# alibaba/nann

Measured on AMD Instinct MI355X. Metric: retrieval QPS @ recall@200 parity, 1M items/128-d, higher is better.
Workload: dtype f16 rows / f32 L2

## Files before the change

### nann_amd/csrc/nann_device.h

```cpp
#pragma once
#include <type_traits>
#include <hip/hip_runtime.h>
#include <hip/hip_fp16.h>
#include <stdint.h>

namespace nann {

constexpr int kNT = 1024;
constexpr int kNW = kNT / 64;
constexpr int kTopkEPT = 16;
constexpr int kMaxK = 1024;
constexpr int kPhaseScratch = 27648;
constexpr int kMaxD = 512;
constexpr int kLdsScoresOff = 10752;
constexpr int kLdsScores = 4096;

enum : int { DT_F16 = 0, DT_BF16 = 1, DT_F32 = 2 };

__device__ __forceinline__ int local_tid() {
  int t = threadIdx.x;
  asm volatile("" : "+v"(t));
  __builtin_assume(t >= 0 && t < 1024);
  return t;
}
// ... 775 lines not shown

template <int DT>
struct RowChunk {
  uint4 a;
  uint4 b;
};

template <int DT>
__device__ __forceinline__ RowChunk<DT> load_chunk(const void* table, size_t row, int d, int sub) {
  RowChunk<DT> r;
  if constexpr (DT == DT_F32) {
    const uint4* p = reinterpret_cast<const uint4*>(static_cast<const float*>(table) + row * d + sub * 8);
    r.a = p[0];
    r.b = p[1];
  } else {
    const uint4* p = reinterpret_cast<const uint4*>(static_cast<const uint16_t*>(table) + row * d + sub * 8);
    r.a = p[0];
    r.b = make_uint4(0, 0, 0, 0);
  }
  return r;
}

template <int DT>
__device__ __forceinline__ void chunk_to_float(const RowChunk<DT>& r, float x[8]) {
  if constexpr (DT == DT_F32) {
    x[0] = __uint_as_float(r.a.x); x[1] = __uint_as_float(r.a.y);
    x[2] = __uint_as_float(r.a.z); x[3] = __uint_as_float(r.a.w);
    x[4] = __uint_as_float(r.b.x); x[5] = __uint_as_float(r.b.y);
    x[6] = __uint_as_float(r.b.z); x[7] = __uint_as_float(r.b.w);
  } else {
    const uint32_t w[4] = {r.a.x, r.a.y, r.a.z, r.a.w};
#pragma unroll
    for (int i = 0; i < 4; ++i) {
      if constexpr (DT == DT_F16) {
        x[2 * i] = half_bits_to_float(w[i] & 0xffffu);
        x[2 * i + 1] = half_bits_to_float(w[i] >> 16);
      } else {
        x[2 * i] = bf16_bits_to_float(w[i] & 0xffffu);
        x[2 * i + 1] = bf16_bits_to_float(w[i] >> 16);
      }
    }
  }
}

template <int LPR>
__device__ __forceinline__ float l2_finish(const float q[8], const float x[8]) {
  float acc = 0.0f;
#pragma unroll
  for (int k = 0; k < 8; ++k) {
    const float t = q[k] - x[k];
    acc = __fmaf_rn(t, t, acc);
  }
  acc = acc + dpp_f32<0xB1>(acc);
  acc = acc + dpp_f32<0x4E>(acc);
  if constexpr (LPR >= 8) acc = acc + dpp_f32<0x141>(acc);
  if constexpr (LPR >= 16) acc = acc + dpp_f32<0x140>(acc);
  if constexpr (LPR >= 32) acc = acc + __shfl_xor(acc, 16);
  if constexpr (LPR >= 64) acc = acc + __shfl_xor(acc, 32);
  return 0.0f - acc;
}

__device__ __forceinline__ float l2_lane_f16(const float q[8], const uint4& a) {
  const uint32_t w[4] = {a.x, a.y, a.z, a.w};
  float acc = 0.0f;
#pragma unroll
  for (int i = 0; i < 4; ++i) {
    float t0, t1;
    asm("v_fma_mix_f32 %0, %1, -1.0, %2 op_sel_hi:[1,0,0]" : "=v"(t0) : "v"(w[i]), "v"(q[2 * i]));
    asm("v_fma_mix_f32 %0, %1, -1.0, %2 op_sel:[1,0,0] op_sel_hi:[1,0,0]" : "=v"(t1) : "v"(w[i]), "v"(q[2 * i + 1]));
    acc = __fmaf_rn(t0, t0, acc);
    acc = __fmaf_rn(t1, t1, acc);
  }
  return acc;
}
__device__ __forceinline__ float l2_lane_bf16(const float q[8], const uint4& a) {
  const uint32_t w[4] = {a.x, a.y, a.z, a.w};
  float acc = 0.0f;
#pragma unroll
  for (int i = 0; i < 4; ++i) {
    const float t0 = q[2 * i] - __uint_as_float(w[i] << 16);
    const float t1 = q[2 * i + 1] - __uint_as_float(w[i] & 0xffff0000u);
    acc = __fmaf_rn(t0, t0, acc);
    acc = __fmaf_rn(t1, t1, acc);
  }
  return acc;
}
__device__ __forceinline__ float l2_rows8_reduce_scatter(float (&a)[8]) {
  float t0, t1, t2, t3;
  asm("s_mov_b32 vcc_lo, 0x5a5a5a5a\n\ts_mov_b32 vcc_hi, 0x5a5a5a5a\n\t"
      "v_cndmask_b32_e32 %8, %0, %1, vcc\n\tv_cndmask_b32_e32 %0, %1, %0, vcc\n\t"
      "v_cndmask_b32_e32 %9, %2, %3, vcc\n\tv_cndmask_b32_e32 %2, %3, %2, vcc\n\t"
      "v_cndmask_b32_e32 %10, %4, %5, vcc\n\tv_cndmask_b32_e32 %4, %5, %4, vcc\n\t"
      "v_cndmask_b32_e32 %11, %6, %7, vcc\n\tv_cndmask_b32_e32 %6, %7, %6, vcc\n\t"
      "v_add_f32_dpp %8, %0, %8 quad_perm:[1,0,3,2] row_mask:0xf bank_mask:0xf\n\t"
      "v_add_f32_dpp %9, %2, %9 quad_perm:[1,0,3,2] row_mask:0xf bank_mask:0xf\n\t"
      "v_add_f32_dpp %10, %4, %10 quad_perm:[1,0,3,2] row_mask:0xf bank_mask:0xf\n\t"
      "v_add_f32_dpp %11, %6, %11 quad_perm:[1,0,3,2] row_mask:0xf bank_mask:0xf\n\t"
      "s_mov_b32 vcc_lo, 0x3c3c3c3c\n\ts_mov_b32 vcc_hi, 0x3c3c3c3c\n\t"
      "v_cndmask_b32_e32 %1, %9, %8, vcc\n\tv_cndmask_b32_e32 %3, %11, %10, vcc\n\t"
      "v_cndmask_b32_e32 %0, %8, %9, vcc\n\tv_cndmask_b32_e32 %2, %10, %11, vcc\n\t"
      "v_add_f32_dpp %0, %1, %0 quad_perm:[2,3,0,1] row_mask:0xf bank_mask:0xf\n\t"
      "v_add_f32_dpp %2, %3, %2 quad_perm:[2,3,0,1] row_mask:0xf bank_mask:0xf\n\t"
      "s_mov_b32 vcc_lo, 0x0ff00ff0\n\ts_mov_b32 vcc_hi, 0x0ff00ff0\n\t"
      "v_cndmask_b32_e32 %8, %2, %0, vcc\n\tv_cndmask_b32_e32 %9, %0, %2, vcc\n\t"
      "s_nop 0\n\t"
      "v_add_f32_dpp %9, %8, %9 row_half_mirror row_mask:0xf bank_mask:0xf\n\t"
      "s_nop 1\n\t"
      "v_add_f32_dpp %9, %9, %9 row_mirror row_mask:0xf bank_mask:0xf"
      : "+v"(a[0]), "+v"(a[1]), "+v"(a[2]), "+v"(a[3]), "+v"(a[4]), "+v"(a[5]), "+v"(a[6]), "+v"(a[7]),
        "=&v"(t0), "=&v"(t1), "=&v"(t2), "=&v"(t3)
      :
      : "vcc");
  return t1;
}

#ifndef NANN_SCORE_U
#define NANN_SCORE_U 8
#endif
#ifndef NANN_SCORE_NT
#define NANN_SCORE_NT 0
#endif
template <int LPR, int DT, int NWAVES>
__device__ __forceinline__ void wg_score_l2_part(const void* __restrict__ table, int d, const int32_t* ids,
                                                 int begin, int end, const float* qv, float* scores,
                                                 int wave_rel, bool near = false) {
  constexpr int U = (DT == DT_F32) ? NANN_SCORE_U / 2 : NANN_SCORE_U;
  constexpr int GPW = 64 / LPR;
  constexpr int RPI = NWAVES * GPW;
  if (end <= begin) return;
  const int lane = local_tid() & 63;
  const int sub = lane % LPR, grp = lane / LPR;
  const int slot = wave_rel * GPW + grp;
  float q[8];
#pragma unroll
  for (int k = 0; k < 8; ++k) q[k] = qv[sub * 8 + k];
  if constexpr (LPR >= 16 && DT != DT_F32) {
    static_assert(U == 8, "eight broadcasts below");
    constexpr uint32_t kRowBytes = LPR * 16;
    const int mine_at = (sub & (U - 1)) * RPI + slot;
    const int out_at = ((sub & 7) ^ ((sub & 4) ? 3 : 0)) * RPI + slot;
    auto run = [&](auto near_c) {
      constexpr bool NEAR = decltype(near_c)::value;
      auto row = [&](int32_t v) -> uint4 {
        if constexpr (NEAR) {
#if NANN_SCORE_NT
          typedef uint32_t u32x4_t __attribute__((ext_vector_type(4)));
          const u32x4_t r = __builtin_nontemporal_load(reinterpret_cast<const u32x4_t*>(static_cast<const unsigned char*>(table) + ((uint32_t)v | ((uint32_t)sub * 16u))));
          return uint4{r.x, r.y, r.z, r.w};
#else
          return *reinterpret_cast<const uint4*>(static_cast<const unsigned char*>(table) + ((uint32_t)v | ((uint32_t)sub * 16u)));
#endif
        } else {
          return load_chunk<DT>(table, (size_t)v, d, sub).a;
        }
      };
      auto widen = [&](int32_t id) -> int32_t { return NEAR ? (int32_t)__umul24((uint32_t)id, kRowBytes) : id; };
      auto ids_of = [&](int at) -> int32_t { return widen(ids[min(at + mine_at, end - 1)]); };
      int32_t idv = ids_of(begin);
      uint4 ch[U];
      ch[0] = row(dpp_i32<0x150>(idv));
      ch[1] = row(dpp_i32<0x151>(idv));
      ch[2] = row(dpp_i32<0x152>(idv));
      ch[3] = row(dpp_i32<0x153>(idv));
      ch[4] = row(dpp_i32<0x154>(idv));
      ch[5] = row(dpp_i32<0x155>(idv));
      ch[6] = row(dpp_i32<0x156>(idv));
      ch[7] = row(dpp_i32<0x157>(idv));
      idv = ids_of(begin + RPI * U);
      auto lane_sum = [&](const uint4& c) -> float { return DT == DT_F16 ? l2_lane_f16(q, c) : l2_lane_bf16(q, c); };
      auto finish = [&](float (&s)[U], int i0) {
        float mine = l2_rows8_reduce_scatter(s);
        if constexpr (LPR >= 32) mine = mine + __shfl_xor(mine, 16);
        if constexpr (LPR >= 64) mine = mine + __shfl_xor(mine, 32);
        const int i = i0 + out_at;
        if (sub < U && i < end) scores[i] = 0.0f - mine;
      };
      int i0 = begin;
      for (; i0 + RPI * U < end; i0 += RPI * U) {
        const int32_t idn = ids_of(i0 + 2 * RPI * U);
        float s[U];
#define NANN_ROLL_SLOT(u, ctrl)                 \
        s[u] = lane_sum(ch[u]);                     \
        ch[u] = row(dpp_i32<ctrl>(idv));            \
        __builtin_amdgcn_sched_barrier(0);
        NANN_ROLL_SLOT(0, 0x150) NANN_ROLL_SLOT(1, 0x151) NANN_ROLL_SLOT(2, 0x152) NANN_ROLL_SLOT(3, 0x153)
        NANN_ROLL_SLOT(4, 0x154) NANN_ROLL_SLOT(5, 0x155) NANN_ROLL_SLOT(6, 0x156) NANN_ROLL_SLOT(7, 0x157)
#undef NANN_ROLL_SLOT
        finish(s, i0);
        idv = idn;
      }
      {
        float s[U];
#pragma unroll
        for (int u = 0; u < U; ++u) s[u] = lane_sum(ch[u]);
        finish(s, i0);
      }
    };
    if (near) run(std::true_type{}); else run(std::false_type{});
    return;
  }
  int32_t nxt[U];
#pragma unroll
  for (int u = 0; u < U; ++u) nxt[u] = ids[min(begin + u * RPI + slot, end - 1)];
  for (int i0 = begin; i0 < end; i0 += RPI * U) {
    RowChunk<DT> ch[U];
#pragma unroll
    for (int u = 0; u < U; ++u) ch[u] = load_chunk<DT>(table, (size_t)nxt[u], d, sub);
#pragma unroll
    for (int u = 0; u < U; ++u)
      nxt[u] = ids[min(i0 + RPI * U + u * RPI + slot, end - 1)];
#pragma unroll
    for (int u = 0; u < U; ++u) {
      const int i = i0 + u * RPI + slot;
      float x[8];
      chunk_to_float<DT>(ch[u], x);
      const float s = l2_finish<LPR>(q, x);
      if (sub == 0 && i < end) scores[i] = s;
    }
  }
}

template <int LPR, int DT, int NTHREADS>
__device__ __forceinline__ void wg_score_l2(const void* __restrict__ table, int d, const int32_t* ids,
                                            int n, const float* qv, float* scores) {
  wg_score_l2_part<LPR, DT, NTHREADS / 64>(table, d, ids, 0, n, qv, scores, local_tid() >> 6);
}

template <int KCAP>
struct TopkScratchT {
  unsigned long long sel[KCAP < 512 ? 512 : KCAP];
  union {
    unsigned short prank[kNT];
    struct { uint32_t above[256]; uint32_t cursor[256]; } bins;
  };
  uint32_t misc[4];
  uint32_t wlo[kNW], whi[kNW];
  uint32_t wcnt[kNW];
};
static_assert(kNT * sizeof(unsigned short) == 512 * sizeof(uint32_t), "the bin tables overlay the partial ranks");
typedef TopkScratchT<kMaxK> TopkScratch;
static_assert(sizeof(TopkScratch) <= kLdsScoresOff, "top-k scratch overlaps the LDS scores");
static_assert(kLdsScoresOff + kLdsScores * 4 <= kPhaseScratch, "phase scratch too small");
static_assert(sizeof(ExpandWalkScratch) <= kPhaseScratch, "phase scratch too small");

template <int NS, bool SCL, int NT, int KCAP = kMaxK, bool BIN = false>
__device__ __forceinline__ int wg_topk_impl(const int32_t* ids, const float* scores,
                                            const float* lds_scores, int n, int k, int32_t* out_pos,
                                            int32_t* out_ids, float* out_scores, const int64_t* id_map,
                                            int64_t* out_mapped, unsigned char* scratch, SubTimer pt,
                                            int n_all = 0x7fffffff, uint32_t floor_key = 0u) {
  TopkScratchT<KCAP>* S = reinterpret_cast<TopkScratchT<KCAP>*>(scratch);
  long long tsub = pt.now();
  const int tid = local_tid(), lane = tid & 63, wave = tid >> 6;
  const uint64_t lt = lanemask_lt(lane);
  constexpr bool REG = NS > 0;
  uint32_t key[REG ? NS : 1];
  if constexpr (REG) {
    float raw[NS];
#pragma unroll
    for (int j = 0; j < NS; ++j) {
      const int i = min(j * NT + tid, n - 1);
      raw[j] = SCL ? lds_scores[i] : scores[i];
    }
#pragma unroll
    for (int j = 0; j < NS; ++j) key[j] = (j * NT + tid < n) ? score_key(raw[j]) : 0u;
  }
#define NANN_FOR_KEYS(...)                                                    \
  if constexpr (REG) {                                                        \
    _Pragma("unroll") for (int j = 0; j < NS; ++j) {                          \
      const int i = j * NT + tid;                                             \
      const uint32_t kj = key[j];                                             \
      const bool valid = i < n && (!BIN || i < n_all || kj > floor_key);      \
      __VA_ARGS__                                                             \
    }                                                                         \
  } else {                                                                    \
    for (int i0 = 0; i0 < n; i0 += NT) {                                      \
      const int i = i0 + tid;                                                 \
// ... 279 lines not shown
```

### nann_amd/csrc/nann_hip.hip

```cpp
#include "nann_eval.h"
#include "nann_attn.h"
#include "nann_order_kernels.h"
#include "host/nann_graphdef_text.h"
#include "host/nann_blaze_options.h"
#include "host/nann_npy.h"
#include "host/nann_projcache.h"

#include <algorithm>
#include <atomic>
#include <cmath>
#include <cstdio>
#include <cstdlib>
#include <cstring>
#include <fstream>
#include <memory>
#include <mutex>
#include <string>
#include <vector>

#include <sys/stat.h>

using namespace nann;

namespace nann {
// ... 2089 lines not shown
    if (cache) projection_used(*cache, tab, st);
    return r2;
  };
  if (attn) {
    a.attn = attn->P;
    if (tab) {
      auto launch = attn->precision == NANN_MLP_SPLIT_F16 ? launch_search_attn_proj : launch_search_attn_xproj;
      const bool resident = attn->precision == NANN_MLP_SPLIT_F16;
      return both([&](int vis, int, int slots, size_t lds) {
        if (resident && vis == VIS_LDS_HASH && !a.redo) return launch_search_attn_res(slots, lds, a, st);
        return launch(vis, slots, lds, a, st);
      });
    }
    auto launch = attn->precision == NANN_MLP_SPLIT_F16 ? launch_search_attn_split : launch_search_attn;
    return both([&](int vis, int, int slots, size_t lds) { return launch(ix->desc.d, dt, vis, slots, lds, a, st); });
  }
  a.mlp = scorer->mlp;
  a.phase = 0;
  const int exact = scorer->desc.kind == NANN_SCORER_MLP && scorer->desc.precision == NANN_MLP_EXACT_F32;
  if (mlp_res && p.phased) {
    DeviceInfo di;
    rc = device_info(&di);
    if (rc) return rc;
    const int k5 = level_topn[5];
    for (int64_t c0 = 0; c0 < n_queries && !rc; c0 += kPhaseChunk) {
      SearchArgs c = a;
      c.n_queries = (int)std::min<int64_t>(kPhaseChunk, n_queries - c0);
      c.q = q + (size_t)c0 * a.d;
      if (tq) c.tq = tq + (size_t)c0 * 6;
      c.out_ids = out_item_ids + (size_t)c0 * k5;
      if (out_scores) c.out_scores = out_scores + (size_t)c0 * k5;
      if (out_index) c.out_index = out_index + (size_t)c0 * k5;
      c.status = status + c0;
      if (counters) c.counters = counters + (size_t)c0 * 3 * NANN_NUM_ROUNDS;
      if (phase_ticks) c.phase_ticks = reinterpret_cast<long long*>(phase_ticks) + (size_t)c0 * NANN_NUM_PHASES;
      if (c0) HIP_TRY(hipMemsetAsync(workspace, 0, 256, st));
      const int slots = (int)std::min<int64_t>(c.n_queries, (int64_t)p.phase_slots);
      for (int ph = 0; ph <= NANN_NUM_ROUNDS && !rc; ++ph) {
        c.phase = ph;
        rc = launch_search_mlp_phase(p.phase_vis, slots, p.phase_lds_bytes, c, st);
        if (!rc && ph < NANN_NUM_ROUNDS) {
          rc = launch_mlp_phase_score(exact, c, ph, p.phase_score_wgs, st);
        }
      }
      if (!rc) {
        c.redo = 1;
        c.phase = 0;
        rc = launch_search_mlp_res(exact, p.fb_vis, p.fb_slots, p.fb_lds_bytes, c, st);
      }
    }
    if (cache) projection_used(*cache, tab, st);
    return rc;
  }
  if (mlp_res)
    return both([&](int vis, int, int slots, size_t lds) {
      return launch_search_mlp_res(exact, vis, slots, lds, a, st);
    });
  return both([&](int vis, int nt, int slots, size_t lds) {
    return launch_search_any(ix->desc.d / 8, dt, kind, mlp_split, vis, nt, slots, lds, a, st);
  });
}

__global__ void k_probe_queries(const void* emb, int dt, int d, long long n_items, int nq, float* q) {
  const int j = blockIdx.x;
  const long long row = (long long)j * (n_items / nq);
  for (int k = threadIdx.x; k < d; k += blockDim.x) {
    float v;
    if (dt == NANN_F32) v = static_cast<const float*>(emb)[row * d + k];
    else {
      const uint32_t h = static_cast<const uint16_t*>(emb)[row * d + k];
      v = dt == NANN_F16 ? half_bits_to_float(h) : bf16_bits_to_float(h);
    }
    q[(size_t)j * d + k] = v;
  }
}

__global__ void k_order_gather(const void* emb, int dt, int d, const int32_t* rows, int m, float* out) {
  for (int k = threadIdx.x; k < d; k += blockDim.x) out[(size_t)blockIdx.x * d + k] = order_row_elem(emb, dt, (size_t)rows[blockIdx.x] * d + k);
}

static int launch_order(const nann_index* ix, const float* q, int n, int32_t* key, int32_t* perm, unsigned int* heads,
                        hipStream_t st) {
  const int d = ix->desc.d, P = ix->n_pivots;
  const size_t lds = ((size_t)d * P + kOrderMaxPivots + (size_t)kOrderKeyQueries * d) * 4;
  if (lds > 48 * 1024)
    HIP_TRY(hipFuncSetAttribute(reinterpret_cast<const void*>(k_order_key), hipFuncAttributeMaxDynamicSharedMemorySize, (int)lds));
  hipLaunchKernelGGL(k_order_key, dim3((unsigned)((n + kOrderKeyQueries - 1) / kOrderKeyQueries)), dim3(256), lds, st,
                     ix->pivots, d, P, q, n, key);
  HIP_TRY(hipGetLastError());
  hipLaunchKernelGGL(k_order_perm, dim3(1), dim3(kOrderSortThreads), 0, st, key, n, P, perm, heads);
  HIP_TRY(hipGetLastError());
  return NANN_OK;
}

static void choose_pivots(nann_index* ix, const std::vector<int32_t>& enter) {
  const int d = ix->desc.d;
  const int P = order_pivots((int64_t)enter.size(), d);
  if (P < 2) return;
  constexpr size_t kMaxCand = 1024;
  const size_t E = enter.size(), m = std::min(E, kMaxCand);
  std::vector<int32_t> cand(m);
  for (size_t i = 0; i < m; ++i) cand[i] = enter[i * E / m];
  int32_t* rows = nullptr;
  float* buf = nullptr;
  std::vector<float> x(m * (size_t)d);
  bool ok = hipMalloc(&rows, m * 4) == hipSuccess && hipMalloc(&buf, m * (size_t)d * 4) == hipSuccess &&
            hipMemcpy(rows, cand.data(), m * 4, hipMemcpyHostToDevice) == hipSuccess;
  if (ok) {
    hipLaunchKernelGGL(k_order_gather, dim3((unsigned)m), dim3(128), 0, nullptr, ix->desc.item_embs, ix->desc.emb_dtype, d, rows, (int)m, buf);
    ok = hipGetLastError() == hipSuccess && hipMemcpy(x.data(), buf, x.size() * 4, hipMemcpyDeviceToHost) == hipSuccess;
  }
  if (buf) (void)hipFree(buf);
  if (rows) (void)hipFree(rows);
  if (!ok) return;
  std::vector<size_t> piv;
  std::vector<double> dist(m, INFINITY);
  size_t cur = 0;
  for (int p = 0; p < P; ++p) {
    piv.push_back(cur);
    size_t far = cur;
    for (size_t i = 0; i < m; ++i) {
      double s = 0.0;
      for (int k = 0; k < d; ++k) { const double t = (double)x[i * d + k] - (double)x[cur * d + k]; s += t * t; }
      dist[i] = std::min(dist[i], s);
      if (dist[i] > dist[far]) far = i;
    }
    if (dist[far] <= 0.0) break;
    cur = far;
  }
  if (piv.size() < 2) return;
  const size_t np = piv.size();
  std::vector<float> t((size_t)d * np + kOrderMaxPivots, 0.0f);
  for (size_t p = 0; p < np; ++p) {
    float s = 0.0f;
    for (int k = 0; k < d; ++k) {
      const float v = x[piv[p] * d + k];
      t[(size_t)k * np + p] = v;
      s += v * v;
    }
    t[(size_t)d * np + p] = s;
  }
  float* dev = nullptr;
  if (hipMalloc(&dev, t.size() * 4) != hipSuccess) return;
  if (hipMemcpy(dev, t.data(), t.size() * 4, hipMemcpyHostToDevice) != hipSuccess) { (void)hipFree(dev); return; }
  ix->pivots = dev;
  ix->n_pivots = (int)piv.size();
}

static void probe_index(nann_index* ix) {
  ix->probe_valid = false;
  static const bool enabled = [] { const char* e = std::getenv("NANN_INDEX_PROBE"); return !(e && e[0] == '0'); }();
  if (!enabled) return;
  const std::string saved_error = nann::g_err;
  struct RestoreError { const std::string& s; ~RestoreError() { nann::g_err = s; } } restore{saved_error};
  const int d = ix->desc.d;
  const int64_t E = ix->desc.n_enter, N = ix->desc.n_items;
  if (E < 8 || N < 4096) return;
  const int nq = 64, e = (int)std::min<int64_t>(64, E);
  const int32_t t[6] = {e, e, e, e, e, std::min(e, 10)};
  nann_scorer_desc sd{};
  sd.kind = NANN_SCORER_L2; sd.d = d; sd.emb_dtype = ix->desc.emb_dtype;
  nann_scorer* sc = nullptr;
  if (nann_scorer_create(&sd, &sc) != NANN_OK) return;
  nann_search_options o;
  nann_search_options_init(&o);
  o.traversal_mode = NANN_TRAVERSAL_HBM_BITMAP;
  o.slot_reserve = 0;
  int64_t ws_bytes = 0;
  const size_t n_ctr = (size_t)nq * 3 * NANN_NUM_ROUNDS;
  unsigned char* buf = nullptr;
  std::vector<int32_t> h_ctr(n_ctr), h_st((size_t)nq);
  bool ok = nann_search_workspace_bytes(ix, t, nq, &ws_bytes) == NANN_OK;
  const size_t off_q = ((size_t)ws_bytes + 255) & ~(size_t)255, off_ids = off_q + (size_t)nq * d * 4,
// ... 429 lines not shown
```

### nann_amd/csrc/nann_order.h

```cpp
#pragma once
#include <hip/hip_runtime.h>
#include <hip/hip_fp16.h>
#include <stdint.h>
#include <algorithm>
#include <cmath>
#include "../../include/nann_hip.h"

namespace nann {

constexpr int kOrderSegs = 8;
constexpr int kOrderHeadStride = 32;
constexpr int kOrderMaxPivots = 128;
constexpr int kOrderPivotLds = 64 * 1024;
constexpr int kOrderKeyQueries = 16;
constexpr int kOrderSortThreads = 1024;

__host__ __device__ inline int order_seg_begin(int n, int s) { return (int)((long long)n * s / kOrderSegs); }

inline int order_pivots(int64_t n_enter, int d) {
  return (int)std::min<int64_t>(n_enter, std::min(kOrderMaxPivots, kOrderPivotLds / (4 * d)));
}

inline unsigned long long order_ws_bytes(int64_t n) {
  return ((unsigned long long)kOrderSegs * kOrderHeadStride * 4 + (unsigned long long)n * 8 + 255) / 256 * 256;
}

__device__ inline unsigned int xcc_id() {
#if defined(__HIP_DEVICE_COMPILE__)
  unsigned int x;
  asm volatile("s_getreg_b32 %0, hwreg(HW_REG_XCC_ID, 0, 4)" : "=s"(x));
  return x;
#else
  return 0;
#endif
}

}
```

### nann_amd/csrc/nann_order_kernels.h

```cpp
#pragma once
#include "nann_order.h"

namespace nann {

__device__ inline float order_row_elem(const void* emb, int dt, size_t i) {
  if (dt == NANN_F32) return reinterpret_cast<const float*>(emb)[i];
  const uint16_t h = reinterpret_cast<const uint16_t*>(emb)[i];
  if (dt == NANN_F16) return __half2float(__ushort_as_half(h));
  return __uint_as_float((uint32_t)h << 16);
}

__global__ __launch_bounds__(256) void k_order_key(const float* pivT, int d, int P, const float* q, int n, int32_t* key) {
  extern __shared__ float4 order_lds4[];
  float* piv = reinterpret_cast<float*>(order_lds4);
  float* qs = piv + (size_t)d * P + kOrderMaxPivots;
  const int q0 = blockIdx.x * kOrderKeyQueries, nq = min(kOrderKeyQueries, n - q0);
  const int pv4 = (d * P + kOrderMaxPivots) / 4, qv4 = nq * d / 4;
  for (int i = threadIdx.x; i < pv4; i += 256) order_lds4[i] = reinterpret_cast<const float4*>(pivT)[i];
  for (int i = threadIdx.x; i < qv4; i += 256)
    reinterpret_cast<float4*>(qs)[i] = reinterpret_cast<const float4*>(q + (size_t)q0 * d)[i];
  __syncthreads();
  const int lane = threadIdx.x & 63, wave = threadIdx.x >> 6;
  const int pa = lane, pb = lane + 64;
  float acc[4][2] = {};
  const float* qw = qs + (size_t)wave * 4 * d;
  for (int k = 0; k < d; ++k) {
    const float va = piv[k * P + min(pa, P - 1)], vb = piv[k * P + min(pb, P - 1)];
#pragma unroll
    for (int j = 0; j < 4; ++j) {
      const float x = qw[j * d + k];
      acc[j][0] = fmaf(x, va, acc[j][0]);
      acc[j][1] = fmaf(x, vb, acc[j][1]);
    }
  }
  const float* pn = piv + (size_t)d * P;
#pragma unroll
  for (int j = 0; j < 4; ++j) {
    const int qi = wave * 4 + j;
    float best = pa < P ? fmaf(-2.0f, acc[j][0], pn[min(pa, P - 1)]) : INFINITY;
    int arg = pa < P ? pa : 0x7fffffff;
    if (pb < P) {
      const float s = fmaf(-2.0f, acc[j][1], pn[pb]);
      if (s < best) { best = s; arg = pb; }
    }
    for (int m = 32; m >= 1; m >>= 1) {
      const float ob = __shfl_xor(best, m);
      const int oa = __shfl_xor(arg, m);
      if (ob < best || (ob == best && oa < arg)) { best = ob; arg = oa; }
    }
    if (lane == 0 && qi < nq) key[q0 + qi] = arg < P ? arg : 0;
  }
}

__global__ __launch_bounds__(kOrderSortThreads) void k_order_perm(const int32_t* key, int n, int P, int32_t* perm,
                                                                 unsigned int* heads) {
  constexpr int W = kOrderSortThreads / 64;
  __shared__ int base[kOrderMaxPivots];
  __shared__ int wofs[W][kOrderMaxPivots];
  const int tid = threadIdx.x, lane = tid & 63, w = tid >> 6;
  if (tid < kOrderSegs * kOrderHeadStride) heads[tid] = 0u;
  for (int p = tid; p < P; p += blockDim.x) base[p] = 0;
  __syncthreads();
  for (int i = tid; i < n; i += blockDim.x) atomicAdd(&base[key[i]], 1);
  __syncthreads();
  int pre = 0;
  if (tid < P)
    for (int p = 0; p < tid; ++p) pre += base[p];
  __syncthreads();
  if (tid < P) base[tid] = pre;
  __syncthreads();
  for (int t0 = 0; t0 < n; t0 += kOrderSortThreads) {
    for (int i = tid; i < W * kOrderMaxPivots; i += blockDim.x) (&wofs[0][0])[i] = 0;
    __syncthreads();
    const int i = t0 + tid;
    const int k = i < n ? key[i] : -1;
    int rank = 0;
    bool last = true;
#pragma unroll
    for (int j = 0; j < 64; ++j) {
      const int kj = __builtin_amdgcn_readlane(k, j);
      if (kj == k) { if (j < lane) ++rank; else if (j > lane) last = false; }
    }
    if (k >= 0 && last) wofs[w][k] = rank + 1;
    __syncthreads();
    for (int p = tid; p < P; p += blockDim.x) {
      int run = base[p];
      for (int v = 0; v < W; ++v) { const int c = wofs[v][p]; wofs[v][p] = run; run += c; }
      base[p] = run;
    }
    __syncthreads();
    if (k >= 0) perm[wofs[w][k] + rank] = i;
    __syncthreads();
  }
}

}
```

Measured before the change: 2.800 million.

## Rewrite query ordering kernels and add optional packed-FMA L2 scoring

Adds a paired-row packed FMA path for f16/bf16 L2 lane sums, gated behind NANN_L2_PK (off by default). The tail block now always goes through lane_pair, which falls back to scalar sums when the flag is off. Separately, k_order_key now handles 32 queries per block, vectorises query loads and the k loop, and reads pivot norms from global memory instead of LDS. k_order_perm is replaced with a per-wave contiguous-range counting sort that uses ballot-based key matching, removing the per-1024-element barrier loop. Together these cut the overhead of query reordering, at the cost of more complex code and higher register use.

Result: faster. 2.834 million (median of 6 runs) (+1.2%).

```diff
diff --git a/nann_amd/csrc/nann_device.h b/nann_amd/csrc/nann_device.h
--- a/nann_amd/csrc/nann_device.h
+++ b/nann_amd/csrc/nann_device.h
@@ -881,6 +881,35 @@
     const float t1 = q[2 * i + 1] - __uint_as_float(w[i] & 0xffff0000u);
     acc = __fmaf_rn(t0, t0, acc);
     acc = __fmaf_rn(t1, t1, acc);
+  }
+  return acc;
+}
+typedef float f32x2_t __attribute__((ext_vector_type(2)));
+__device__ __forceinline__ f32x2_t l2_lane_f16_pair(const float q[8], const uint4& a, const uint4& b) {
+  const uint32_t wa[4] = {a.x, a.y, a.z, a.w}, wb[4] = {b.x, b.y, b.z, b.w};
+  f32x2_t acc = {0.0f, 0.0f};
+#pragma unroll
+  for (int i = 0; i < 4; ++i) {
+    float a0, a1, b0, b1;
+    asm("v_fma_mix_f32 %0, %1, -1.0, %2 op_sel_hi:[1,0,0]" : "=v"(a0) : "v"(wa[i]), "v"(q[2 * i]));
+    asm("v_fma_mix_f32 %0, %1, -1.0, %2 op_sel_hi:[1,0,0]" : "=v"(b0) : "v"(wb[i]), "v"(q[2 * i]));
+    asm("v_fma_mix_f32 %0, %1, -1.0, %2 op_sel:[1,0,0] op_sel_hi:[1,0,0]" : "=v"(a1) : "v"(wa[i]), "v"(q[2 * i + 1]));
+    asm("v_fma_mix_f32 %0, %1, -1.0, %2 op_sel:[1,0,0] op_sel_hi:[1,0,0]" : "=v"(b1) : "v"(wb[i]), "v"(q[2 * i + 1]));
+    const f32x2_t t0 = {a0, b0}, t1 = {a1, b1};
+    acc = __builtin_elementwise_fma(t0, t0, acc);
+    acc = __builtin_elementwise_fma(t1, t1, acc);
+  }
+  return acc;
+}
+__device__ __forceinline__ f32x2_t l2_lane_bf16_pair(const float q[8], const uint4& a, const uint4& b) {
+  const uint32_t wa[4] = {a.x, a.y, a.z, a.w}, wb[4] = {b.x, b.y, b.z, b.w};
+  f32x2_t acc = {0.0f, 0.0f};
+#pragma unroll
+  for (int i = 0; i < 4; ++i) {
+    const f32x2_t t0 = {q[2 * i] - __uint_as_float(wa[i] << 16), q[2 * i] - __uint_as_float(wb[i] << 16)};
+    const f32x2_t t1 = {q[2 * i + 1] - __uint_as_float(wa[i] & 0xffff0000u), q[2 * i + 1] - __uint_as_float(wb[i] & 0xffff0000u)};
+    acc = __builtin_elementwise_fma(t0, t0, acc);
+    acc = __builtin_elementwise_fma(t1, t1, acc);
   }
   return acc;
 }
@@ -918,6 +947,9 @@
 #endif
 #ifndef NANN_SCORE_NT
 #define NANN_SCORE_NT 0
+#endif
+#ifndef NANN_L2_PK
+#define NANN_L2_PK 0
 #endif
 template <int LPR, int DT, int NWAVES>
 __device__ __forceinline__ void wg_score_l2_part(const void* __restrict__ table, int d, const int32_t* ids,
@@ -967,6 +999,16 @@
       ch[7] = row(dpp_i32<0x157>(idv));
       idv = ids_of(begin + RPI * U);
       auto lane_sum = [&](const uint4& c) -> float { return DT == DT_F16 ? l2_lane_f16(q, c) : l2_lane_bf16(q, c); };
+      auto lane_pair = [&](float (&s)[U], int u) {
+        if constexpr (NANN_L2_PK) {
+          const f32x2_t p = DT == DT_F16 ? l2_lane_f16_pair(q, ch[u], ch[u + 1]) : l2_lane_bf16_pair(q, ch[u], ch[u + 1]);
+          s[u] = p.x;
+          s[u + 1] = p.y;
+        } else {
+          s[u] = lane_sum(ch[u]);
+          s[u + 1] = lane_sum(ch[u + 1]);
+        }
+      };
       auto finish = [&](float (&s)[U], int i0) {
         float mine = l2_rows8_reduce_scatter(s);
         if constexpr (LPR >= 32) mine = mine + __shfl_xor(mine, 16);
@@ -978,6 +1020,16 @@
       for (; i0 + RPI * U < end; i0 += RPI * U) {
         const int32_t idn = ids_of(i0 + 2 * RPI * U);
         float s[U];
+#if NANN_L2_PK
+#define NANN_ROLL_PAIR(u, c0, c1)               \
+        lane_pair(s, u);                            \
+        ch[u] = row(dpp_i32<c0>(idv));              \
+        ch[u + 1] = row(dpp_i32<c1>(idv));          \
+        __builtin_amdgcn_sched_barrier(0);
+        NANN_ROLL_PAIR(0, 0x150, 0x151) NANN_ROLL_PAIR(2, 0x152, 0x153)
+        NANN_ROLL_PAIR(4, 0x154, 0x155) NANN_ROLL_PAIR(6, 0x156, 0x157)
+#undef NANN_ROLL_PAIR
+#else
 #define NANN_ROLL_SLOT(u, ctrl)                 \
         s[u] = lane_sum(ch[u]);                     \
         ch[u] = row(dpp_i32<ctrl>(idv));            \
@@ -985,13 +1037,14 @@
         NANN_ROLL_SLOT(0, 0x150) NANN_ROLL_SLOT(1, 0x151) NANN_ROLL_SLOT(2, 0x152) NANN_ROLL_SLOT(3, 0x153)
         NANN_ROLL_SLOT(4, 0x154) NANN_ROLL_SLOT(5, 0x155) NANN_ROLL_SLOT(6, 0x156) NANN_ROLL_SLOT(7, 0x157)
 #undef NANN_ROLL_SLOT
+#endif
         finish(s, i0);
         idv = idn;
       }
       {
         float s[U];
 #pragma unroll
-        for (int u = 0; u < U; ++u) s[u] = lane_sum(ch[u]);
+        for (int u = 0; u < U; u += 2) lane_pair(s, u);
         finish(s, i0);
       }
     };
diff --git a/nann_amd/csrc/nann_hip.hip b/nann_amd/csrc/nann_hip.hip
--- a/nann_amd/csrc/nann_hip.hip
+++ b/nann_amd/csrc/nann_hip.hip
@@ -2195,7 +2195,7 @@
 static int launch_order(const nann_index* ix, const float* q, int n, int32_t* key, int32_t* perm, unsigned int* heads,
                         hipStream_t st) {
   const int d = ix->desc.d, P = ix->n_pivots;
-  const size_t lds = ((size_t)d * P + kOrderMaxPivots + (size_t)kOrderKeyQueries * d) * 4;
+  const size_t lds = ((size_t)d * P + (size_t)kOrderKeyQueries * d) * 4;
   if (lds > 48 * 1024)
     HIP_TRY(hipFuncSetAttribute(reinterpret_cast<const void*>(k_order_key), hipFuncAttributeMaxDynamicSharedMemorySize, (int)lds));
   hipLaunchKernelGGL(k_order_key, dim3((unsigned)((n + kOrderKeyQueries - 1) / kOrderKeyQueries)), dim3(256), lds, st,
diff --git a/nann_amd/csrc/nann_order.h b/nann_amd/csrc/nann_order.h
--- a/nann_amd/csrc/nann_order.h
+++ b/nann_amd/csrc/nann_order.h
@@ -12,8 +12,9 @@
 constexpr int kOrderHeadStride = 32;
 constexpr int kOrderMaxPivots = 128;
 constexpr int kOrderPivotLds = 64 * 1024;
-constexpr int kOrderKeyQueries = 16;
+constexpr int kOrderKeyQueries = 32;
 constexpr int kOrderSortThreads = 1024;
+constexpr int kOrderSortChunks = 4;
 
 __host__ __device__ inline int order_seg_begin(int n, int s) { return (int)((long long)n * s / kOrderSegs); }
 
diff --git a/nann_amd/csrc/nann_order_kernels.h b/nann_amd/csrc/nann_order_kernels.h
--- a/nann_amd/csrc/nann_order_kernels.h
+++ b/nann_amd/csrc/nann_order_kernels.h
@@ -11,33 +11,53 @@
 }
 
 __global__ __launch_bounds__(256) void k_order_key(const float* pivT, int d, int P, const float* q, int n, int32_t* key) {
+  constexpr int QW = kOrderKeyQueries / 4;
+  constexpr int PU = kOrderPivotLds / (16 * 256), QU = 4;
   extern __shared__ float4 order_lds4[];
   float* piv = reinterpret_cast<float*>(order_lds4);
-  float* qs = piv + (size_t)d * P + kOrderMaxPivots;
+  float* qs = piv + (size_t)d * P;
   const int q0 = blockIdx.x * kOrderKeyQueries, nq = min(kOrderKeyQueries, n - q0);
-  const int pv4 = (d * P + kOrderMaxPivots) / 4, qv4 = nq * d / 4;
-  for (int i = threadIdx.x; i < pv4; i += 256) order_lds4[i] = reinterpret_cast<const float4*>(pivT)[i];
-  for (int i = threadIdx.x; i < qv4; i += 256)
-    reinterpret_cast<float4*>(qs)[i] = reinterpret_cast<const float4*>(q + (size_t)q0 * d)[i];
+  const int pv4 = d * P / 4, qv4 = nq * d / 4;
+  typedef float f32x4_t __attribute__((ext_vector_type(4)));
+  const f32x4_t* psrc = reinterpret_cast<const f32x4_t*>(pivT);
+  const f32x4_t* qsrc = reinterpret_cast<const f32x4_t*>(q + (size_t)q0 * d);
+  f32x4_t* pdst = reinterpret_cast<f32x4_t*>(piv);
+  f32x4_t* qdst = reinterpret_cast<f32x4_t*>(qs);
+  {
+    f32x4_t rp[PU], rq[QU];
+#pragma unroll
+    for (int u = 0; u < PU; ++u) rp[u] = psrc[min((int)threadIdx.x + 256 * u, pv4 - 1)];
+#pragma unroll
+    for (int u = 0; u < QU; ++u) rq[u] = qsrc[min((int)threadIdx.x + 256 * u, qv4 - 1)];
+#pragma unroll
+    for (int u = 0; u < PU; ++u) pdst[min((int)threadIdx.x + 256 * u, pv4 - 1)] = rp[u];
+#pragma unroll
+    for (int u = 0; u < QU; ++u) qdst[min((int)threadIdx.x + 256 * u, qv4 - 1)] = rq[u];
+  }
+  for (int i = threadIdx.x + 256 * QU; i < qv4; i += 256) qdst[i] = qsrc[i];
   __syncthreads();
   const int lane = threadIdx.x & 63, wave = threadIdx.x >> 6;
-  const int pa = lane, pb = lane + 64;
-  float acc[4][2] = {};
-  const float* qw = qs + (size_t)wave * 4 * d;
-  for (int k = 0; k < d; ++k) {
-    const float va = piv[k * P + min(pa, P - 1)], vb = piv[k * P + min(pb, P - 1)];
+  const int pa = lane, pb = lane + 64, ia = min(pa, P - 1), ib = min(pb, P - 1);
+  float acc[QW][2] = {};
+  const float* qw = qs + (size_t)wave * QW * d;
+  for (int k = 0; k < d; k += 4) {
+    float va[4], vb[4];
 #pragma unroll
-    for (int j = 0; j < 4; ++j) {
-      const float x = qw[j * d + k];
-      acc[j][0] = fmaf(x, va, acc[j][0]);
-      acc[j][1] = fmaf(x, vb, acc[j][1]);
+    for (int t = 0; t < 4; ++t) { va[t] = piv[(k + t) * P + ia]; vb[t] = piv[(k + t) * P + ib]; }
+#pragma unroll
+    for (int j = 0; j < QW; ++j) {
+      const float4 x = *reinterpret_cast<const float4*>(qw + j * d + k);
+      acc[j][0] = fmaf(x.x, va[0], acc[j][0]); acc[j][1] = fmaf(x.x, vb[0], acc[j][1]);
+      acc[j][0] = fmaf(x.y, va[1], acc[j][0]); acc[j][1] = fmaf(x.y, vb[1], acc[j][1]);
+      acc[j][0] = fmaf(x.z, va[2], acc[j][0]); acc[j][1] = fmaf(x.z, vb[2], acc[j][1]);
+      acc[j][0] = fmaf(x.w, va[3], acc[j][0]); acc[j][1] = fmaf(x.w, vb[3], acc[j][1]);
     }
   }
-  const float* pn = piv + (size_t)d * P;
+  const float* pn = pivT + (size_t)d * P;
 #pragma unroll
-  for (int j = 0; j < 4; ++j) {
-    const int qi = wave * 4 + j;
-    float best = pa < P ? fmaf(-2.0f, acc[j][0], pn[min(pa, P - 1)]) : INFINITY;
+  for (int j = 0; j < QW; ++j) {
+    const int qi = wave * QW + j;
+    float best = pa < P ? fmaf(-2.0f, acc[j][0], pn[ia]) : INFINITY;
     int arg = pa < P ? pa : 0x7fffffff;
     if (pb < P) {
       const float s = fmaf(-2.0f, acc[j][1], pn[pb]);
@@ -52,45 +72,69 @@
   }
 }
 
+__device__ inline uint64_t order_match(int k, bool valid) {
+  uint64_t m = __ballot(valid);
+#pragma unroll
+  for (int b = 0; (1 << b) < kOrderMaxPivots; ++b) {
+    const bool set = (k >> b) & 1;
+    const uint64_t v = __ballot(set);
+    m &= set ? v : ~v;
+  }
+  return m;
+}
+
 __global__ __launch_bounds__(kOrderSortThreads) void k_order_perm(const int32_t* key, int n, int P, int32_t* perm,
                                                                  unsigned int* heads) {
-  constexpr int W = kOrderSortThreads / 64;
+  constexpr int W = kOrderSortThreads / 64, C = kOrderSortChunks;
   __shared__ int base[kOrderMaxPivots];
-  __shared__ int wofs[W][kOrderMaxPivots];
+  __shared__ int cnt[W][kOrderMaxPivots];
   const int tid = threadIdx.x, lane = tid & 63, w = tid >> 6;
   if (tid < kOrderSegs * kOrderHeadStride) heads[tid] = 0u;
-  for (int p = tid; p < P; p += blockDim.x) base[p] = 0;
+  for (int i = tid; i < W * kOrderMaxPivots; i += kOrderSortThreads) (&cnt[0][0])[i] = 0;
   __syncthreads();
-  for (int i = tid; i < n; i += blockDim.x) atomicAdd(&base[key[i]], 1);
+  const int lo = (int)((long long)n * w / W), hi = (int)((long long)n * (w + 1) / W);
+  const uint64_t below = (1ull << lane) - 1;
+  for (int c = lo; c < hi; c += 64 * C) {
+    int k[C];
+#pragma unroll
+    for (int u = 0; u < C; ++u) k[u] = c + 64 * u + lane < hi ? key[c + 64 * u + lane] : 0;
+#pragma unroll
+    for (int u = 0; u < C; ++u) {
+      const bool v = c + 64 * u + lane < hi;
+      const uint64_t m = order_match(k[u], v);
+      if (v && (m & below) == 0) cnt[w][k[u]] += __popcll(m);
+    }
+  }
   __syncthreads();
-  int pre = 0;
-  if (tid < P)
-    for (int p = 0; p < tid; ++p) pre += base[p];
+  if (tid < P) {
+    int run = 0;
+    for (int v = 0; v < W; ++v) { const int c = cnt[v][tid]; cnt[v][tid] = run; run += c; }
+    base[tid] = run;
+  }
   __syncthreads();
-  if (tid < P) base[tid] = pre;
+  if (w == 0) {
+    const int a = 2 * lane < P ? base[2 * lane] : 0, b = 2 * lane + 1 < P ? base[2 * lane + 1] : 0;
+    int s = a + b;
+    for (int o = 1; o < 64; o <<= 1) {
+      const int t = __shfl_up(s, o);
+      if (lane >= o) s += t;
+    }
+    if (2 * lane < P) base[2 * lane] = s - a - b;
+    if (2 * lane + 1 < P) base[2 * lane + 1] = s - b;
+  }
   __syncthreads();
-  for (int t0 = 0; t0 < n; t0 += kOrderSortThreads) {
-    for (int i = tid; i < W * kOrderMaxPivots; i += blockDim.x) (&wofs[0][0])[i] = 0;
-    __syncthreads();
-    const int i = t0 + tid;
-    const int k = i < n ? key[i] : -1;
-    int rank = 0;
-    bool last = true;
+  for (int c = lo; c < hi; c += 64 * C) {
+    int k[C];
 #pragma unroll
-    for (int j = 0; j < 64; ++j) {
-      const int kj = __builtin_amdgcn_readlane(k, j);
-      if (kj == k) { if (j < lane) ++rank; else if (j > lane) last = false; }
+    for (int u = 0; u < C; ++u) k[u] = c + 64 * u + lane < hi ? key[c + 64 * u + lane] : 0;
+#pragma unroll
+    for (int u = 0; u < C; ++u) {
+      const int i = c + 64 * u + lane;
+      const bool v = i < hi;
+      const uint64_t m = order_match(k[u], v);
+      if (v) perm[base[k[u]] + cnt[w][k[u]] + __popcll(m & below)] = i;
+      if (v && (m & below) == 0) cnt[w][k[u]] += __popcll(m);
     }
-    if (k >= 0 && last) wofs[w][k] = rank + 1;
-    __syncthreads();
-    for (int p = tid; p < P; p += blockDim.x) {
-      int run = base[p];
-      for (int v = 0; v < W; ++v) { const int c = wofs[v][p]; wofs[v][p] = run; run += c; }
-      base[p] = run;
-    }
-    __syncthreads();
-    if (k >= 0) perm[wofs[w][k] + rank] = i;
-    __syncthreads();
   }
 }
 
```

## Pack paired-row L2 with v_pk_fma and rewrite order key/perm kernels

Applied to the files above, without the earlier changes.

The gather-scoring loop now scores two rows at once with packed f32 ops (v_pk_mul/v_pk_fma, v_pk_add for bf16), cutting VALU instruction count in the distance inner loop. The pivot-key kernel stages its pivot and query loads through registers and unrolls the d loop by 8. The permutation kernel is rewritten as a tiled counting sort that finds equal keys with ballot bit-matching instead of 64 readlanes, processes 4 keys per thread, and uses a shuffle-based scan. The changes touch unrelated kernels, and the new sort assumes at most 128 pivots.

New measurement: 2.800 million before, 2.881 million after (median of 6 runs). 2.9% higher.

```diff
diff --git a/nann_amd/csrc/nann_device.h b/nann_amd/csrc/nann_device.h
--- a/nann_amd/csrc/nann_device.h
+++ b/nann_amd/csrc/nann_device.h
@@ -881,6 +881,42 @@
     const float t1 = q[2 * i + 1] - __uint_as_float(w[i] & 0xffff0000u);
     acc = __fmaf_rn(t0, t0, acc);
     acc = __fmaf_rn(t1, t1, acc);
+  }
+  return acc;
+}
+
+typedef float l2x2_t __attribute__((ext_vector_type(2)));
+__device__ __forceinline__ void l2_sq_acc2(l2x2_t& acc, l2x2_t t, bool first) {
+  if (first) asm("v_pk_mul_f32 %0, %1, %1" : "=v"(acc) : "v"(t));
+  else asm("v_pk_fma_f32 %0, %1, %1, %0" : "+v"(acc) : "v"(t));
+}
+__device__ __forceinline__ l2x2_t l2_lane2_f16(const float q[8], const uint4& a, const uint4& b) {
+  const uint32_t wa[4] = {a.x, a.y, a.z, a.w}, wb[4] = {b.x, b.y, b.z, b.w};
+  l2x2_t acc;
+#pragma unroll
+  for (int i = 0; i < 4; ++i) {
+    float ta0, tb0, ta1, tb1;
+    asm("v_fma_mix_f32 %0, %1, -1.0, %2 op_sel_hi:[1,0,0]" : "=v"(ta0) : "v"(wa[i]), "v"(q[2 * i]));
+    asm("v_fma_mix_f32 %0, %1, -1.0, %2 op_sel_hi:[1,0,0]" : "=v"(tb0) : "v"(wb[i]), "v"(q[2 * i]));
+    l2_sq_acc2(acc, l2x2_t{ta0, tb0}, i == 0);
+    asm("v_fma_mix_f32 %0, %1, -1.0, %2 op_sel:[1,0,0] op_sel_hi:[1,0,0]" : "=v"(ta1) : "v"(wa[i]), "v"(q[2 * i + 1]));
+    asm("v_fma_mix_f32 %0, %1, -1.0, %2 op_sel:[1,0,0] op_sel_hi:[1,0,0]" : "=v"(tb1) : "v"(wb[i]), "v"(q[2 * i + 1]));
+    l2_sq_acc2(acc, l2x2_t{ta1, tb1}, false);
+  }
+  return acc;
+}
+__device__ __forceinline__ l2x2_t l2_lane2_bf16(const l2x2_t qp[4], const uint4& a, const uint4& b) {
+  const uint32_t wa[4] = {a.x, a.y, a.z, a.w}, wb[4] = {b.x, b.y, b.z, b.w};
+  l2x2_t acc;
+#pragma unroll
+  for (int i = 0; i < 4; ++i) {
+    l2x2_t t0, t1;
+    asm("v_pk_add_f32 %0, %1, %2 op_sel_hi:[0,1] neg_lo:[0,1] neg_hi:[0,1]"
+        : "=v"(t0) : "v"(qp[i]), "v"(l2x2_t{__uint_as_float(wa[i] << 16), __uint_as_float(wb[i] << 16)}));
+    l2_sq_acc2(acc, t0, i == 0);
+    asm("v_pk_add_f32 %0, %1, %2 op_sel:[1,0] op_sel_hi:[1,1] neg_lo:[0,1] neg_hi:[0,1]"
+        : "=v"(t1) : "v"(qp[i]), "v"(l2x2_t{__uint_as_float(wa[i] & 0xffff0000u), __uint_as_float(wb[i] & 0xffff0000u)}));
+    l2_sq_acc2(acc, t1, false);
   }
   return acc;
 }
@@ -966,7 +1002,12 @@
       ch[6] = row(dpp_i32<0x156>(idv));
       ch[7] = row(dpp_i32<0x157>(idv));
       idv = ids_of(begin + RPI * U);
-      auto lane_sum = [&](const uint4& c) -> float { return DT == DT_F16 ? l2_lane_f16(q, c) : l2_lane_bf16(q, c); };
+      const l2x2_t qp[4] = {{q[0], q[1]}, {q[2], q[3]}, {q[4], q[5]}, {q[6], q[7]}};
+      auto pair_sum = [&](float (&s)[U], int u) {
+        const l2x2_t p = DT == DT_F16 ? l2_lane2_f16(q, ch[u], ch[u + 1]) : l2_lane2_bf16(qp, ch[u], ch[u + 1]);
+        s[u] = p.x;
+        s[u + 1] = p.y;
+      };
       auto finish = [&](float (&s)[U], int i0) {
         float mine = l2_rows8_reduce_scatter(s);
         if constexpr (LPR >= 32) mine = mine + __shfl_xor(mine, 16);
@@ -978,20 +1019,21 @@
       for (; i0 + RPI * U < end; i0 += RPI * U) {
         const int32_t idn = ids_of(i0 + 2 * RPI * U);
         float s[U];
-#define NANN_ROLL_SLOT(u, ctrl)                 \
-        s[u] = lane_sum(ch[u]);                     \
-        ch[u] = row(dpp_i32<ctrl>(idv));            \
+#define NANN_ROLL_PAIR(u, ctrl0, ctrl1)         \
+        pair_sum(s, u);                             \
+        ch[u] = row(dpp_i32<ctrl0>(idv));           \
+        ch[u + 1] = row(dpp_i32<ctrl1>(idv));       \
         __builtin_amdgcn_sched_barrier(0);
-        NANN_ROLL_SLOT(0, 0x150) NANN_ROLL_SLOT(1, 0x151) NANN_ROLL_SLOT(2, 0x152) NANN_ROLL_SLOT(3, 0x153)
-        NANN_ROLL_SLOT(4, 0x154) NANN_ROLL_SLOT(5, 0x155) NANN_ROLL_SLOT(6, 0x156) NANN_ROLL_SLOT(7, 0x157)
-#undef NANN_ROLL_SLOT
+        NANN_ROLL_PAIR(0, 0x150, 0x151) NANN_ROLL_PAIR(2, 0x152, 0x153)
+        NANN_ROLL_PAIR(4, 0x154, 0x155) NANN_ROLL_PAIR(6, 0x156, 0x157)
+#undef NANN_ROLL_PAIR
         finish(s, i0);
         idv = idn;
       }
       {
         float s[U];
 #pragma unroll
-        for (int u = 0; u < U; ++u) s[u] = lane_sum(ch[u]);
+        for (int u = 0; u < U; u += 2) pair_sum(s, u);
         finish(s, i0);
       }
     };
diff --git a/nann_amd/csrc/nann_hip.hip b/nann_amd/csrc/nann_hip.hip
--- a/nann_amd/csrc/nann_hip.hip
+++ b/nann_amd/csrc/nann_hip.hip
@@ -2201,7 +2201,7 @@
   hipLaunchKernelGGL(k_order_key, dim3((unsigned)((n + kOrderKeyQueries - 1) / kOrderKeyQueries)), dim3(256), lds, st,
                      ix->pivots, d, P, q, n, key);
   HIP_TRY(hipGetLastError());
-  hipLaunchKernelGGL(k_order_perm, dim3(1), dim3(kOrderSortThreads), 0, st, key, n, P, perm, heads);
+  hipLaunchKernelGGL(k_order_perm, dim3(1), dim3(kOrderSortThreads), 0, st, key, n, perm, heads);
   HIP_TRY(hipGetLastError());
   return NANN_OK;
 }
diff --git a/nann_amd/csrc/nann_order.h b/nann_amd/csrc/nann_order.h
--- a/nann_amd/csrc/nann_order.h
+++ b/nann_amd/csrc/nann_order.h
@@ -13,7 +13,10 @@
 constexpr int kOrderMaxPivots = 128;
 constexpr int kOrderPivotLds = 64 * 1024;
 constexpr int kOrderKeyQueries = 16;
+constexpr int kOrderMaxD = 512;
 constexpr int kOrderSortThreads = 1024;
+constexpr int kOrderSortE = 4;
+constexpr int kOrderSortTile = kOrderSortThreads * kOrderSortE;
 
 __host__ __device__ inline int order_seg_begin(int n, int s) { return (int)((long long)n * s / kOrderSegs); }
 
diff --git a/nann_amd/csrc/nann_order_kernels.h b/nann_amd/csrc/nann_order_kernels.h
--- a/nann_amd/csrc/nann_order_kernels.h
+++ b/nann_amd/csrc/nann_order_kernels.h
@@ -10,33 +10,49 @@
   return __uint_as_float((uint32_t)h << 16);
 }
 
-__global__ __launch_bounds__(256) void k_order_key(const float* pivT, int d, int P, const float* q, int n, int32_t* key) {
+__global__ __launch_bounds__(256) void k_order_key(const float* __restrict__ pivT, int d, int P, const float* __restrict__ q,
+                                                   int n, int32_t* __restrict__ key) {
   extern __shared__ float4 order_lds4[];
   float* piv = reinterpret_cast<float*>(order_lds4);
-  float* qs = piv + (size_t)d * P + kOrderMaxPivots;
-  const int q0 = blockIdx.x * kOrderKeyQueries, nq = min(kOrderKeyQueries, n - q0);
-  const int pv4 = (d * P + kOrderMaxPivots) / 4, qv4 = nq * d / 4;
-  for (int i = threadIdx.x; i < pv4; i += 256) order_lds4[i] = reinterpret_cast<const float4*>(pivT)[i];
-  for (int i = threadIdx.x; i < qv4; i += 256)
-    reinterpret_cast<float4*>(qs)[i] = reinterpret_cast<const float4*>(q + (size_t)q0 * d)[i];
+  constexpr int kStage = (kOrderPivotLds + kOrderMaxPivots * 4 + 16 * 256 - 1) / (16 * 256);
+  constexpr int kStageQ = (kOrderKeyQueries * kOrderMaxD * 4 + 16 * 256 - 1) / (16 * 256);
+  const int pv4 = (d * P + kOrderMaxPivots) / 4, qv4 = kOrderKeyQueries * d / 4;
+  const int q0 = blockIdx.x * kOrderKeyQueries;
+  const float4* qsrc = reinterpret_cast<const float4*>(q);
+  const float4* qsrc_wg = qsrc + (size_t)min(q0, n - 1) * d / 4;
+  const int qv4_wg = min(qv4, (n - min(q0, n - 1)) * d / 4);
+  float4 stage[kStage], stq[kStageQ];
+#pragma unroll
+  for (int r = 0; r < kStage; ++r) stage[r] = reinterpret_cast<const float4*>(pivT)[min((int)threadIdx.x + r * 256, pv4 - 1)];
+#pragma unroll
+  for (int r = 0; r < kStageQ; ++r) stq[r] = qsrc_wg[min((int)threadIdx.x + r * 256, qv4_wg - 1)];
+#pragma unroll
+  for (int r = 0; r < kStage; ++r) order_lds4[min((int)threadIdx.x + r * 256, pv4 - 1)] = stage[r];
+#pragma unroll
+  for (int r = 0; r < kStageQ; ++r) order_lds4[pv4 + min((int)threadIdx.x + r * 256, qv4 - 1)] = stq[r];
   __syncthreads();
   const int lane = threadIdx.x & 63, wave = threadIdx.x >> 6;
   const int pa = lane, pb = lane + 64;
+  const float* qw = piv + (size_t)pv4 * 4 + (size_t)wave * 4 * d;
   float acc[4][2] = {};
-  const float* qw = qs + (size_t)wave * 4 * d;
-  for (int k = 0; k < d; ++k) {
-    const float va = piv[k * P + min(pa, P - 1)], vb = piv[k * P + min(pb, P - 1)];
+  const float* ca = piv + min(pa, P - 1);
+  const float* cb = piv + min(pb, P - 1);
+  for (int k0 = 0; k0 < d; k0 += 8) {
+    float va[8], vb[8];
 #pragma unroll
-    for (int j = 0; j < 4; ++j) {
-      const float x = qw[j * d + k];
-      acc[j][0] = fmaf(x, va, acc[j][0]);
-      acc[j][1] = fmaf(x, vb, acc[j][1]);
-    }
+    for (int k = 0; k < 8; ++k) { va[k] = ca[(k0 + k) * P]; vb[k] = cb[(k0 + k) * P]; }
+#pragma unroll
+    for (int j = 0; j < 4; ++j)
+#pragma unroll
+      for (int k = 0; k < 8; ++k) {
+        const float x = qw[j * d + k0 + k];
+        acc[j][0] = fmaf(x, va[k], acc[j][0]);
+        acc[j][1] = fmaf(x, vb[k], acc[j][1]);
+      }
   }
   const float* pn = piv + (size_t)d * P;
 #pragma unroll
   for (int j = 0; j < 4; ++j) {
-    const int qi = wave * 4 + j;
     float best = pa < P ? fmaf(-2.0f, acc[j][0], pn[min(pa, P - 1)]) : INFINITY;
     int arg = pa < P ? pa : 0x7fffffff;
     if (pb < P) {
@@ -48,48 +64,107 @@
       const int oa = __shfl_xor(arg, m);
       if (ob < best || (ob == best && oa < arg)) { best = ob; arg = oa; }
     }
-    if (lane == 0 && qi < nq) key[q0 + qi] = arg < P ? arg : 0;
+    const int qi = q0 + wave * 4 + j;
+    if (lane == 0 && qi < n) key[qi] = arg < P ? arg : 0;
   }
 }
 
-__global__ __launch_bounds__(kOrderSortThreads) void k_order_perm(const int32_t* key, int n, int P, int32_t* perm,
-                                                                 unsigned int* heads) {
-  constexpr int W = kOrderSortThreads / 64;
+__global__ __launch_bounds__(kOrderSortThreads) void k_order_perm(const int32_t* __restrict__ key, int n, int32_t* __restrict__ perm,
+                                                                 unsigned int* __restrict__ heads) {
+  constexpr int W = kOrderSortThreads / 64, E = kOrderSortE, S = E * W;
+  constexpr int G = kOrderSortThreads / kOrderMaxPivots;
+  static_assert(S % G == 0 && G <= 64 && (G & (G - 1)) == 0 && kOrderMaxPivots == 128, "scan layout");
+  __shared__ int cnt[kOrderMaxPivots * S];
+  __shared__ int tot[kOrderMaxPivots];
   __shared__ int base[kOrderMaxPivots];
-  __shared__ int wofs[W][kOrderMaxPivots];
   const int tid = threadIdx.x, lane = tid & 63, w = tid >> 6;
   if (tid < kOrderSegs * kOrderHeadStride) heads[tid] = 0u;
-  for (int p = tid; p < P; p += blockDim.x) base[p] = 0;
-  __syncthreads();
-  for (int i = tid; i < n; i += blockDim.x) atomicAdd(&base[key[i]], 1);
-  __syncthreads();
-  int pre = 0;
-  if (tid < P)
-    for (int p = 0; p < tid; ++p) pre += base[p];
-  __syncthreads();
-  if (tid < P) base[tid] = pre;
-  __syncthreads();
-  for (int t0 = 0; t0 < n; t0 += kOrderSortThreads) {
-    for (int i = tid; i < W * kOrderMaxPivots; i += blockDim.x) (&wofs[0][0])[i] = 0;
+  const int tiles = (n + kOrderSortTile - 1) / kOrderSortTile;
+  int kk[E], rk[E];
+  auto load = [&](int t0) {
+#pragma unroll
+    for (int e = 0; e < E; ++e) {
+      const int i = t0 + e * kOrderSortThreads + tid;
+      kk[e] = i < n ? key[i] : -1;
+    }
+  };
+  auto match = [&](int e) -> int {
+    const int k = kk[e];
+    unsigned long long peers = __ballot(k >= 0);
+#pragma unroll
+    for (int b = 0; b < 7; ++b) {
+      const unsigned long long bal = __ballot((k >> b) & 1);
+      peers &= ((k >> b) & 1) ? bal : ~bal;
+    }
+    rk[e] = __popcll(peers & ((1ull << lane) - 1ull));
+    return (k >= 0 && (peers >> lane) == 1ull) ? __popcll(peers) : 0;
+  };
+  auto scan_keys = [&](const int* src, int* dst) {
+    if (w == 0) {
+      const int a = src[2 * lane], b = src[2 * lane + 1];
+      int x = a + b;
+#pragma unroll
+      for (int o = 1; o < 64; o <<= 1) {
+        const int y = __shfl_up(x, o);
+        if (lane >= o) x += y;
+      }
+      x -= a + b;
+      dst[2 * lane] = x;
+      dst[2 * lane + 1] = x + a;
+    }
+  };
+  if (tiles > 1) {
+    if (tid < kOrderMaxPivots) tot[tid] = 0;
     __syncthreads();
-    const int i = t0 + tid;
-    const int k = i < n ? key[i] : -1;
-    int rank = 0;
-    bool last = true;
+    for (int t = 0; t < tiles; ++t) {
+      load(t * kOrderSortTile);
 #pragma unroll
-    for (int j = 0; j < 64; ++j) {
-      const int kj = __builtin_amdgcn_readlane(k, j);
-      if (kj == k) { if (j < lane) ++rank; else if (j > lane) last = false; }
-    }
-    if (k >= 0 && last) wofs[w][k] = rank + 1;
-    __syncthreads();
-    for (int p = tid; p < P; p += blockDim.x) {
-      int run = base[p];
-      for (int v = 0; v < W; ++v) { const int c = wofs[v][p]; wofs[v][p] = run; run += c; }
-      base[p] = run;
+      for (int e = 0; e < E; ++e) {
+        const int c = match(e);
+        if (c) atomicAdd(&tot[kk[e]], c);
+      }
     }
     __syncthreads();
-    if (k >= 0) perm[wofs[w][k] + rank] = i;
+    scan_keys(tot, base);
+  }
+  for (int t = 0; t < tiles; ++t) {
+    const int t0 = t * kOrderSortTile;
+    load(t0);
+    for (int i = tid; i < kOrderMaxPivots * S / 4; i += kOrderSortThreads) reinterpret_cast<int4*>(cnt)[i] = make_int4(0, 0, 0, 0);
+    __syncthreads();
+#pragma unroll
+    for (int e = 0; e < E; ++e) {
+      const int c = match(e);
+      if (c) cnt[kk[e] * S + e * W + w] = c;
+    }
+    __syncthreads();
+    const int p = tid / G, g = tid % G;
+    constexpr int C = S / G;
+    int c[C], run = 0;
+#pragma unroll
+    for (int i = 0; i < C; ++i) { c[i] = run; run += cnt[p * S + g * C + i]; }
+    int gx = run;
+#pragma unroll
+    for (int o = 1; o < G; o <<= 1) {
+      const int y = __shfl_up(gx, o);
+      if (g >= o) gx += y;
+    }
+    const int key_tot = __shfl(gx, (lane & ~(G - 1)) + G - 1);
+    gx -= run;
+    if (tiles == 1) {
+      if (g == 0) tot[p] = key_tot;
+      __syncthreads();
+      scan_keys(tot, base);
+      __syncthreads();
+    }
+    const int b0 = base[p] + gx;
+#pragma unroll
+    for (int i = 0; i < C; ++i) cnt[p * S + g * C + i] = b0 + c[i];
+    if (g == G - 1) base[p] += key_tot;
+    __syncthreads();
+#pragma unroll
+    for (int e = 0; e < E; ++e)
+      if (kk[e] >= 0) perm[cnt[kk[e] * S + e * W + w] + rk[e]] = t0 + e * kOrderSortThreads + tid;
     __syncthreads();
   }
 }
```
